# caumente/multi_task_breast_cancer

Hardware: AMD Instinct MI355X
Metric: training images/sec (1-ch 256x256, U-Net++ MT) (higher is better)
Workload: dtype bf16; 1 GPU; MTUNetPlusPlus seg+cls deep-supervision step (Dice+Focal, alpha=0.5, Adam eps 1e-4), per-GPU batch 32, 1x256x256, bf16 MFMA operands (3x3 convs, ConvT) and 16-bit stored conv outputs / activations; fp32 accumulation, gradient sums, statistics, losses, parameters and optimizer, random-init weights (BASELINE.json configs[1]); global_batch=32, parallelism=dp1

## Files before the change

### include/mtbc.h

```cpp
#ifndef MTBC_H
#define MTBC_H

#include <stddef.h>
#include <stdint.h>

#ifdef __cplusplus
extern "C" {
#endif

#define MTBC_VERSION 202
#define MTBC_MAX_SEGS 6

enum {
    MTBC_OK = 0,
    MTBC_E_BADSHAPE = -1,
    MTBC_E_BADARG = -2,
    MTBC_E_WORKSPACE = -3,
    MTBC_E_LAUNCH = -4,
    MTBC_E_UNSUPPORTED = -5
};

int mtbc_version(void);
const char* mtbc_strerror(int code);
const char* mtbc_arch(void);
// ... 163 lines not shown
    int32_t accumulate_dw;
    void* workspace; size_t workspace_bytes;
    int32_t compute;
    int32_t y_layout;
    int32_t y_type;
    int32_t x_layout;
    int32_t dy_type16;
    int32_t x_type16;
} mtbc_convT_args;
int mtbc_convT_fwd_c8_supported(const mtbc_convT_args* a);

size_t mtbc_convT_wgrad_workspace(const mtbc_convT_args* a);
int mtbc_convT_fwd(const mtbc_convT_args* a, void* stream);
int mtbc_convT_dgrad(const mtbc_convT_args* a, void* stream);
int mtbc_convT_wgrad(const mtbc_convT_args* a, void* stream);

typedef struct {
    int32_t N, H, W, Cin, Cout;
    const float* x;  int64_t x_batch_stride;
    const float* w;
    const float* bias;
    float* y;
    const float* dy;
    float* dx;       int64_t dx_batch_stride;
    int32_t accumulate_dx;
    float* dw;       float* dbias;
    int32_t accumulate_dw;
    void* workspace; size_t workspace_bytes;
    int32_t x_layout;
    int32_t x_type;
// ... 179 lines not shown
```

### multi_task_breast_cancer_amd/_lib.py

```python
from __future__ import annotations

import ctypes as C
import os
from typing import Optional

_HERE = os.path.dirname(os.path.abspath(__file__))
LIB_PATH = os.environ.get("MTBC_LIB") or os.path.join(_HERE, "libmtbc_hip.so")

MAX_SEGS = 6
c_float_p = C.POINTER(C.c_float)


class MtbcError(RuntimeError):
    pass


LAYOUT_PLANAR, LAYOUT_C8 = 0, 1


class Seg(C.Structure):
    _fields_ = [("ptr", C.c_void_p), ("batch_stride", C.c_int64), ("channels", C.c_int32), ("accumulate", C.c_int32)]


class Conv3x3Args(C.Structure):
# ... 194 lines not shown
    _fields_ = [("w", C.c_void_p), ("packed", C.c_void_p), ("Cin", C.c_int32), ("Cout", C.c_int32),
                ("kind", C.c_int32), ("compute", C.c_int32)]


class WViewDesc(C.Structure):
    _fields_ = [("w", C.c_void_p), ("dst", C.c_void_p), ("Cout", C.c_int32), ("Cin", C.c_int32), ("ci_off", C.c_int32),
                ("ci_cnt", C.c_int32), ("mode", C.c_int32), ("k_off", C.c_int32), ("K", C.c_int32)]


EXPORTS = [
    "mtbc_version", "mtbc_strerror", "mtbc_arch",
    "mtbc_conv3x3_packed_elems", "mtbc_conv3x3_packed_dgrad_elems", "mtbc_conv3x3_pack_fwd",
    "mtbc_conv3x3_pack_dgrad", "mtbc_conv3x3_packed_lp_elems", "mtbc_conv3x3_pack_lp", "mtbc_conv3x3_pack_many", "mtbc_c8_pack", "mtbc_c8_unpack", "mtbc_c8_pack16", "mtbc_conv3x3_weight_view", "mtbc_conv3x3_weight_view_many", "mtbc_augment_flip_rotate", "mtbc_convT_head_combine", "mtbc_convT_head_expand", "mtbc_conv3x3_wgrad_workspace", "mtbc_conv3x3_wgrad_sync_bytes", "mtbc_conv3x3_stats_slots", "mtbc_conv3x3_kernel_name", "mtbc_conv3x3_fwd", "mtbc_conv3x3_dgrad",
    "mtbc_conv3x3_wgrad", "mtbc_instnorm_fwd_workspace", "mtbc_instnorm_coop_state_bytes", "mtbc_instnorm_coop_error_offset", "mtbc_instnorm_c8_supported", "mtbc_instnorm_bwd_team", "mtbc_instnorm_dparam_many", "mtbc_instnorm_lrelu_fwd", "mtbc_instnorm_lrelu_bwd", "mtbc_maxpool2_fwd",
    "mtbc_maxpool2_bwd", "mtbc_convT_wgrad_workspace", "mtbc_convT_fwd_c8_supported", "mtbc_convT_fwd", "mtbc_convT_dgrad", "mtbc_convT_wgrad",
    "mtbc_conv1x1_wgrad_workspace", "mtbc_conv1x1_fwd", "mtbc_conv1x1_dgrad", "mtbc_conv1x1_wgrad",
    "mtbc_gap_fwd", "mtbc_gap_bwd", "mtbc_linear_fwd", "mtbc_linear_bwd", "mtbc_dice_fwd", "mtbc_dice_bwd",
    "mtbc_focal_fwd_bwd", "mtbc_loss_mix", "mtbc_adam_step", "mtbc_adam_dynamic", "mtbc_loss_scale_begin", "mtbc_loss_scale_check", "mtbc_loss_scale_adam",
    "mtbc_loss_scale_update_host", "mtbc_loss_scale_begin_host", "mtbc_dice_counts", "mtbc_program_run",
    "mtbc_program_run_ms", "mtbc_event_create", "mtbc_event_destroy",
    "mtbc_seg_metrics_workspace_size", "mtbc_seg_metrics",
]

ABI_VERSION = 202
_lib: Optional[C.CDLL] = None


def load() -> C.CDLL:
    global _lib
    if _lib is not None:
# ... 32 lines not shown
    lib.mtbc_c8_pack.restype = C.c_int
    lib.mtbc_c8_pack.argtypes = [C.c_void_p, C.c_int64, C.c_void_p, C.c_int32, C.c_int32, C.c_int32, C.c_int32, C.c_void_p]
    lib.mtbc_conv3x3_weight_view.restype = C.c_int
    lib.mtbc_conv3x3_weight_view.argtypes = [C.c_void_p, C.c_void_p] + [C.c_int32] * 7 + [C.c_void_p]
    lib.mtbc_conv3x3_weight_view_many.restype = C.c_int
    lib.mtbc_conv3x3_weight_view_many.argtypes = [C.POINTER(WViewDesc), C.c_int32, C.c_void_p]
    lib.mtbc_c8_pack16.restype = C.c_int
    lib.mtbc_c8_pack16.argtypes = [C.c_void_p, C.c_int64, C.c_void_p, C.c_int32, C.c_int32, C.c_int32, C.c_void_p]
    lib.mtbc_c8_unpack.restype = C.c_int
    lib.mtbc_c8_unpack.argtypes = [C.c_void_p, C.c_void_p, C.c_int32, C.c_int32, C.c_int32, C.c_int32, C.c_void_p]
    lib.mtbc_conv3x3_pack_lp.restype = C.c_int
    lib.mtbc_conv3x3_pack_lp.argtypes = [C.c_void_p, C.c_void_p, C.c_int32, C.c_int32, C.c_int32, C.c_int32, C.c_void_p]
    for name in ("mtbc_conv3x3_pack_fwd", "mtbc_conv3x3_pack_dgrad"):
        getattr(lib, name).restype = C.c_int
        getattr(lib, name).argtypes = [C.c_void_p, C.c_void_p, C.c_int32, C.c_int32, C.c_void_p]
    for name, typ in (("mtbc_conv3x3_wgrad_workspace", Conv3x3Args), ("mtbc_conv3x3_wgrad_sync_bytes", Conv3x3Args), ("mtbc_convT_wgrad_workspace", ConvTArgs),
                      ("mtbc_conv1x1_wgrad_workspace", Conv1x1Args)):
        getattr(lib, name).restype = C.c_size_t
        getattr(lib, name).argtypes = [C.POINTER(typ)]
    for name, typ in (("mtbc_conv3x3_fwd", Conv3x3Args), ("mtbc_conv3x3_dgrad", Conv3x3Args),
                      ("mtbc_conv3x3_wgrad", Conv3x3Args), ("mtbc_instnorm_lrelu_fwd", InstNormArgs),
                      ("mtbc_instnorm_lrelu_bwd", InstNormArgs), ("mtbc_maxpool2_fwd", MaxPoolArgs),
                      ("mtbc_maxpool2_bwd", MaxPoolArgs), ("mtbc_convT_fwd", ConvTArgs),
                      ("mtbc_convT_dgrad", ConvTArgs), ("mtbc_convT_wgrad", ConvTArgs),
                      ("mtbc_conv1x1_fwd", Conv1x1Args), ("mtbc_conv1x1_dgrad", Conv1x1Args),
                      ("mtbc_conv1x1_wgrad", Conv1x1Args), ("mtbc_gap_fwd", GapArgs), ("mtbc_gap_bwd", GapArgs),
                      ("mtbc_linear_fwd", LinearArgs), ("mtbc_linear_bwd", LinearArgs),
                      ("mtbc_dice_fwd", DiceArgs), ("mtbc_dice_bwd", DiceArgs), ("mtbc_focal_fwd_bwd", FocalArgs),
                      ("mtbc_adam_step", AdamArgs)):
        getattr(lib, name).restype = C.c_int
        getattr(lib, name).argtypes = [C.POINTER(typ), C.c_void_p]
    lib.mtbc_instnorm_coop_state_bytes.restype = C.c_size_t
    lib.mtbc_instnorm_coop_state_bytes.argtypes = []
    lib.mtbc_instnorm_coop_error_offset.restype = C.c_size_t
    lib.mtbc_instnorm_coop_error_offset.argtypes = []
    lib.mtbc_instnorm_bwd_team.restype = C.c_int32
    lib.mtbc_instnorm_bwd_team.argtypes = [C.POINTER(InstNormArgs)]
    lib.mtbc_instnorm_dparam_many.restype = C.c_int
    lib.mtbc_instnorm_dparam_many.argtypes = [C.POINTER(DparamDesc), C.c_int32, C.c_void_p]
    lib.mtbc_instnorm_c8_supported.restype = C.c_int
    lib.mtbc_instnorm_c8_supported.argtypes = [C.POINTER(InstNormArgs), C.c_int32]
    lib.mtbc_convT_fwd_c8_supported.restype = C.c_int
    lib.mtbc_convT_fwd_c8_supported.argtypes = [C.POINTER(ConvTArgs)]
    lib.mtbc_loss_mix.restype = C.c_int
    lib.mtbc_loss_mix.argtypes = [C.c_void_p, C.c_void_p, C.c_float, C.c_void_p, C.c_void_p]
    lib.mtbc_dice_counts.restype = C.c_int
    lib.mtbc_dice_counts.argtypes = [C.c_void_p, C.c_void_p, C.c_int64, C.c_void_p, C.c_void_p]
    lib.mtbc_adam_dynamic.restype = C.c_int
    lib.mtbc_adam_dynamic.argtypes = [C.POINTER(AdamArgs), C.POINTER(C.c_float * 3)]
    for name in ("mtbc_loss_scale_begin", "mtbc_loss_scale_check"):
        getattr(lib, name).restype = C.c_int
        getattr(lib, name).argtypes = [C.POINTER(LossScaleArgs), C.c_void_p]
    lib.mtbc_loss_scale_adam.restype = C.c_int
    lib.mtbc_loss_scale_adam.argtypes = [C.POINTER(LossScaleArgs), C.POINTER(AdamArgs), C.c_void_p]
    for name in ("mtbc_loss_scale_update_host", "mtbc_loss_scale_begin_host"):
        getattr(lib, name).restype = C.c_int
        getattr(lib, name).argtypes = [C.POINTER(LossScaleArgs)]
    lib.mtbc_program_run.restype = C.c_int
# ... 27 lines not shown
```

### multi_task_breast_cancer_amd/csrc/common.h

```cpp
#pragma once
#include <hip/hip_runtime.h>
#include <stdint.h>
#include "../../include/mtbc.h"

#define MTBC_WAVE 64

typedef float f32x4 __attribute__((ext_vector_type(4)));

#define MTBC_CHECK_LAUNCH()                                   \
    do {                                                      \
        hipError_t e__ = hipGetLastError();                   \
        if (e__ != hipSuccess) return MTBC_E_LAUNCH;          \
    } while (0)

#ifdef MTBC_PROBES
#include <stdlib.h>
static inline int mtbc_probe_int(const char* name, int dflt) { const char* v = getenv(name); return v ? atoi(v) : dflt; }
static inline bool mtbc_probe_set(const char* name) { return getenv(name) != nullptr; }
#define MTBC_DBG_BIT(p, bit) ((p).dbg & (bit))
#else
#define mtbc_probe_int(name, dflt) (dflt)
#define mtbc_probe_set(name) (false)
#define MTBC_DBG_BIT(p, bit) (0)
#endif
// ... 100 lines not shown
int mtbc_i_maxpool_c8_bwd(const mtbc_maxpool_args* a, hipStream_t st);
int mtbc_i_conv1x1_c8_fwd(const mtbc_conv1x1_args* a, hipStream_t st);
size_t mtbc_i_conv1x1_c8_wgrad_workspace(const mtbc_conv1x1_args* a);
int mtbc_i_conv1x1_c8_wgrad(const mtbc_conv1x1_args* a, hipStream_t st);
int mtbc_i_splitk_reduce(const float* partial, float* out, int nsplit, size_t elems, int accumulate, hipStream_t st);
int mtbc_i_splitk_reduce2(const float* partial, float* out, float* out2, int nsplit, size_t elems1, size_t elems2, int accumulate, hipStream_t st);
bool mtbc_i_convT2_fwd_ok(const mtbc_convT_args* a);
int mtbc_i_convT2_fwd(const mtbc_convT_args* a, hipStream_t st);
bool mtbc_i_convT2_fwd_c8_ok(const mtbc_convT_args* a);
int mtbc_i_convT2_fwd_c8(const mtbc_convT_args* a, hipStream_t st);
bool mtbc_i_convT2_fwd_lp_c8_ok(const mtbc_convT_args* a);
int mtbc_i_convT2_fwd_lp_c8(const mtbc_convT_args* a, hipStream_t st);
bool mtbc_i_convT2_dgrad_ok(const mtbc_convT_args* a);
bool mtbc_i_convT2_wgrad_ok(const mtbc_convT_args* a);
void mtbc_i_convT2_wgrad_plan(const mtbc_convT_args* a, int* steps_per_split, int* nsplit);
int mtbc_i_convT2_dgrad(const mtbc_convT_args* a, int compute, hipStream_t st);
int mtbc_i_convT2_wgrad(const mtbc_convT_args* a, int compute, float* partial, float* dbias_part, int steps_per_split, int nsplit, hipStream_t st);
int mtbc_i_channel_sums(const float* x, float* planes_ws, float* out, int N, int C, int HW, int accumulate, hipStream_t st);
```

### multi_task_breast_cancer_amd/csrc/convt2.hip

```cpp
#include "common.h"
#include <utility>

namespace {

typedef __bf16 bf16x8 __attribute__((ext_vector_type(8)));
typedef _Float16 f16x8 __attribute__((ext_vector_type(8)));

template <int LP> struct Frag;
template <> struct Frag<0> {
    float v[8];
    __device__ __forceinline__ void set(const float* f) {
#pragma unroll
        for (int i = 0; i < 8; ++i) v[i] = f[i];
    }
    static __device__ __forceinline__ f32x4 mma(const Frag& a, const Frag& b, f32x4 c) {
#pragma unroll
        for (int i = 0; i < 8; ++i) c = __builtin_amdgcn_mfma_f32_16x16x4f32(a.v[i], b.v[i], c, 0, 0, 0);
        return c;
    }
};
template <> struct Frag<1> {
    bf16x8 v;
    __device__ __forceinline__ void set(const float* f) {
#pragma unroll
// ... 770 lines not shown
            for (int m = 0; m < MT; ++m)
#pragma unroll
                for (int r = 0; r < 4; ++r) old[m][r] = *reinterpret_cast<const float2*>(dxn + (size_t)min(mb * 48 + m * 16 + kg * 4 + r, p.Cin - 1) * HW);
        }
#pragma unroll
        for (int m = 0; m < MT; ++m)
#pragma unroll
            for (int r = 0; r < 4; ++r) {
                const int ci = mb * 48 + m * 16 + kg * 4 + r;
                if (ci >= p.Cin) continue;
                float2 v = make_float2(acc[m][0][r], acc[m][1][r]);
                if (p.acc_dx) { v.x += old[m][r].x; v.y += old[m][r].y; }
                *reinterpret_cast<float2*>(dxn + (size_t)ci * HW) = v;
            }
    }
}

bool al16(const void* q) { return (reinterpret_cast<uintptr_t>(q) & 15) == 0; }

void fill(const mtbc_convT_args* a, Ct2P* p) {
    p->N = a->N; p->H = a->H; p->W = a->W; p->Cin = a->Cin; p->Cout = a->Cout;
    p->x = a->x; p->xbs = a->x_batch_stride; p->w = a->w; p->dy = a->dy; p->dybs = a->dy_batch_stride;
    p->dx = a->dx; p->dxbs = a->dx_batch_stride; p->acc_dx = a->accumulate_dx; p->partial = nullptr; p->dbias_part = nullptr;
    p->mblocks = cdiv(a->Cin, 48); p->ctiles = cdiv(a->Cout, 8); p->steps_per_split = 1; p->nsplit = 1; p->ntasks = 0; p->xcd_tasks = 0;
}

}

bool mtbc_i_convT2_dgrad_ok(const mtbc_convT_args* a) {
    const int HW = a->H * a->W;
// ... 169 lines not shown
            else hipLaunchKernelGGL((convT2_wgrad16_kernel<2, 2, 4>), dim3(b2), dim3(256), 0, st, p);
        } else {
            const unsigned b1 = xblocks ? xblocks : blocks;
            if (compute == 1) hipLaunchKernelGGL((convT2_wgrad16_kernel<1, 1, 4>), dim3(b1), dim3(256), 0, st, p);
            else hipLaunchKernelGGL((convT2_wgrad16_kernel<2, 1, 4>), dim3(b1), dim3(256), 0, st, p);
        }
    } else if (a->dy_type16) {
        if (compute == 1) hipLaunchKernelGGL((convT2_wgrad_kernel<1, true>), dim3(blocks), dim3(256), 0, st, p);
        else hipLaunchKernelGGL((convT2_wgrad_kernel<2, true>), dim3(blocks), dim3(256), 0, st, p);
    } else if (compute == 1) hipLaunchKernelGGL(convT2_wgrad_kernel<1>, dim3(blocks), dim3(256), 0, st, p);
    else if (compute == 2) hipLaunchKernelGGL(convT2_wgrad_kernel<2>, dim3(blocks), dim3(256), 0, st, p);
    else hipLaunchKernelGGL(convT2_wgrad_kernel<0>, dim3(blocks), dim3(256), 0, st, p);
    MTBC_CHECK_LAUNCH();
    return MTBC_OK;
}
```

### multi_task_breast_cancer_amd/csrc/pool_up.hip

```cpp
#include "common.h"
#include <cstdlib>

namespace {

constexpr int GRS = 81;

template <bool A_KCONTIG, bool B_KCONTIG, class AL, class BL, class CS>
__device__ __forceinline__ void gemm_block_64x64(int m0, int c0, int kbeg, int kend, AL al, BL bl, CS cs) {
    constexpr int BK = 32;
    __shared__ float As[BK * GRS];
    __shared__ float Bs[BK * GRS];
    const int tid = threadIdx.x, lane = tid & 63, wv = tid >> 6;
    const int j = lane & 15, kk = lane >> 4;
    const int mrow = 32 * (wv >> 1), ccol = 32 * (wv & 1);
    f32x4 acc[2][2];
#pragma unroll
    for (int a = 0; a < 2; ++a)
#pragma unroll
        for (int b = 0; b < 2; ++b) acc[a][b] = (f32x4){0.f, 0.f, 0.f, 0.f};

    float ra[8], rb[8];
    auto fetch = [&](int k0) {
#pragma unroll
        for (int i = 0; i < 8; ++i) {
// ... 356 lines not shown
        if (a->k == 2) hipLaunchKernelGGL(convT_wgrad_kernel<2>, grid, dim3(256), 0, st, p);
        else if (a->k == 4) hipLaunchKernelGGL(convT_wgrad_kernel<4>, grid, dim3(256), 0, st, p);
        else hipLaunchKernelGGL(convT_wgrad_kernel<8>, grid, dim3(256), 0, st, p);
        MTBC_CHECK_LAUNCH();
    }
    const size_t wel = (size_t)a->Cin * p.M;
    rc = mtbc_i_splitk_reduce(p.partial, a->dw, nsplit, wel, a->accumulate_dw, st); if (rc) return rc;
    if (a->dbias && !bias_done) {
        if (p.dybs != (long long)a->Cout * a->H * a->W * a->k * a->k) return MTBC_E_UNSUPPORTED;
        rc = mtbc_i_channel_sums(p.dy, p.partial + (size_t)nsplit * wel, a->dbias, a->N, a->Cout, a->H * a->W * a->k * a->k,
                                 a->accumulate_dw, st);
        if (rc) return rc;
    }
    return MTBC_OK;
}

static int fill_mp(const mtbc_maxpool_args* a, MpP* p) {
    if (!a || a->N <= 0 || a->C <= 0 || a->H < 2 || a->W < 2 || (a->H & 1) || (a->W & 1)) return MTBC_E_BADSHAPE;
    p->N = a->N; p->C = a->C; p->H = a->H; p->W = a->W; p->x = a->x; p->xbs = a->x_batch_stride; p->y = a->y;
    p->ybs = a->y_batch_stride; p->dy = a->dy; p->dybs = a->dy_batch_stride; p->dx = a->dx; p->dxbs = a->dx_batch_stride;
    p->acc = a->accumulate_dx;
    return MTBC_OK;
}
int mtbc_maxpool2_fwd(const mtbc_maxpool_args* a, void* stream) {
    MpP p; int rc = fill_mp(a, &p); if (rc) return rc;
    if (!p.x || !p.y) return MTBC_E_BADARG;
    if (a->layout == MTBC_LAYOUT_C8) return mtbc_i_maxpool_c8_fwd(a, (hipStream_t)stream);
    if (a->layout != MTBC_LAYOUT_PLANAR) return MTBC_E_BADARG;
    hipStream_t st = (hipStream_t)stream;
    if ((a->W & 3) == 0 && al16(p.x) && (p.xbs & 3) == 0 && (reinterpret_cast<uintptr_t>(p.y) & 7) == 0 && (p.ybs & 1) == 0) {
// ... 144 lines not shown
```

### multi_task_breast_cancer_amd/csrc/program.hip

```cpp
#include "common.h"

extern "C" {

int mtbc_version(void) { return MTBC_VERSION; }
const char* mtbc_arch(void) { return "gfx950"; }

const char* mtbc_strerror(int code) {
    switch (code) {
        case MTBC_OK: return "ok";
        case MTBC_E_BADSHAPE: return "bad shape";
        case MTBC_E_BADARG: return "bad argument (null or misaligned pointer)";
        case MTBC_E_WORKSPACE: return "workspace missing or too small";
        case MTBC_E_LAUNCH: return "kernel launch failed";
        case MTBC_E_UNSUPPORTED: return "unsupported configuration";
        default: return "unknown error";
    }
}

static inline bool is_pack(int32_t k) { return k == MTBC_OP_CONV3_PACK_FWD || k == MTBC_OP_CONV3_PACK_DGRAD || k == MTBC_OP_CONV3_PACK_LP; }

int mtbc_event_create(void** event) {
    if (!event) return MTBC_E_BADARG;
    hipEvent_t e;
    if (hipEventCreateWithFlags(&e, hipEventDisableTiming) != hipSuccess) return MTBC_E_LAUNCH;
// ... 78 lines not shown
            case MTBC_OP_CONV3_WGRAD: rc = mtbc_conv3x3_wgrad(&o->u.conv3, stream); break;
            case MTBC_OP_CONV3_PACK_FWD: rc = mtbc_conv3x3_pack_fwd(o->u.pack.w, o->u.pack.packed, o->u.pack.Cin, o->u.pack.Cout, stream); break;
            case MTBC_OP_CONV3_PACK_DGRAD: rc = mtbc_conv3x3_pack_dgrad(o->u.pack.w, o->u.pack.packed, o->u.pack.Cin, o->u.pack.Cout, stream); break;
            case MTBC_OP_HEAD_COMBINE: rc = mtbc_convT_head_combine(&o->u.head, stream); break;
            case MTBC_OP_HEAD_EXPAND: rc = mtbc_convT_head_expand(&o->u.head, stream); break;
            case MTBC_OP_CONV3_WVIEW: rc = mtbc_conv3x3_weight_view(o->u.wview.w, o->u.wview.dst, o->u.wview.Cout, o->u.wview.Cin, o->u.wview.ci_off, o->u.wview.ci_cnt, o->u.wview.mode, o->u.wview.k_off, o->u.wview.K, stream); break;
            case MTBC_OP_C8_PACK16: rc = mtbc_c8_pack16(o->u.c8pack.src, o->u.c8pack.src_batch_stride, o->u.c8pack.dst, o->u.c8pack.N, o->u.c8pack.C, o->u.c8pack.HW, stream); break;
            case MTBC_OP_C8_PACK: rc = mtbc_c8_pack(o->u.c8pack.src, o->u.c8pack.src_batch_stride, o->u.c8pack.dst, o->u.c8pack.N, o->u.c8pack.C, o->u.c8pack.HW, o->u.c8pack.compute, stream); break;
            case MTBC_OP_CONV3_PACK_LP: rc = mtbc_conv3x3_pack_lp(o->u.pack.w, o->u.pack.packed, o->u.pack.Cin, o->u.pack.Cout, o->u.pack.dgrad, o->u.pack.compute, stream); break;
            case MTBC_OP_IN_FWD: rc = mtbc_instnorm_lrelu_fwd(&o->u.inorm, stream); break;
            case MTBC_OP_IN_BWD: rc = mtbc_instnorm_lrelu_bwd(&o->u.inorm, stream); break;
            case MTBC_OP_POOL_FWD: rc = mtbc_maxpool2_fwd(&o->u.pool, stream); break;
            case MTBC_OP_POOL_BWD: rc = mtbc_maxpool2_bwd(&o->u.pool, stream); break;
            case MTBC_OP_CONVT_FWD: rc = mtbc_convT_fwd(&o->u.convT, stream); break;
            case MTBC_OP_CONVT_DGRAD: rc = mtbc_convT_dgrad(&o->u.convT, stream); break;
            case MTBC_OP_CONVT_WGRAD: rc = mtbc_convT_wgrad(&o->u.convT, stream); break;
            case MTBC_OP_CONV1_FWD: rc = mtbc_conv1x1_fwd(&o->u.conv1, stream); break;
            case MTBC_OP_CONV1_DGRAD: rc = mtbc_conv1x1_dgrad(&o->u.conv1, stream); break;
            case MTBC_OP_CONV1_WGRAD: rc = mtbc_conv1x1_wgrad(&o->u.conv1, stream); break;
            case MTBC_OP_GAP_FWD: rc = mtbc_gap_fwd(&o->u.gap, stream); break;
            case MTBC_OP_GAP_BWD: rc = mtbc_gap_bwd(&o->u.gap, stream); break;
            case MTBC_OP_LINEAR_FWD: rc = mtbc_linear_fwd(&o->u.linear, stream); break;
            case MTBC_OP_LINEAR_BWD: rc = mtbc_linear_bwd(&o->u.linear, stream); break;
            case MTBC_OP_DICE_FWD: rc = mtbc_dice_fwd(&o->u.dice, stream); break;
            case MTBC_OP_DICE_BWD: rc = mtbc_dice_bwd(&o->u.dice, stream); break;
            case MTBC_OP_FOCAL: rc = mtbc_focal_fwd_bwd(&o->u.focal, stream); break;
            case MTBC_OP_LOSS_MIX: rc = mtbc_loss_mix(o->u.mix.seg, o->u.mix.cls, o->u.mix.alpha, o->u.mix.out4, stream); break;
            case MTBC_OP_ADAM: rc = mtbc_adam_step(&o->u.adam, stream); break;
            case MTBC_OP_MEMSET:
                rc = hipMemsetAsync(o->u.memset0.ptr, 0, o->u.memset0.bytes, (hipStream_t)stream) == hipSuccess ? MTBC_OK : MTBC_E_LAUNCH;
                break;
// ... 13 lines not shown
```

### multi_task_breast_cancer_amd/engine.py

```python
from __future__ import annotations

import ctypes as C
from dataclasses import dataclass, field
from typing import Callable, Dict, List, Optional, Sequence, Tuple

import torch

from . import _lib as L


from . import switches as _sw

_sw.refuse_removed()
_NO_COOP = _sw.flag("MTBC_NO_COOP")
_NO_GATHER = _sw.flag("MTBC_NO_GATHER")
_NO_Z16 = _sw.flag("MTBC_NO_Z16")
_Z_BF16 = _sw.flag("MTBC_Z_BF16")
_DA16 = _sw.flag("MTBC_DA16")
_COOP_MIN_FWD, _COOP_MIN_BWD = 16384, 65536
_IN_KERNEL_SPLITK = False
_DPARAM_BATCH = 12


def _ptr(t: Optional[torch.Tensor]) -> Optional[int]:
    return None if t is None else t.data_ptr()


@dataclass
class Act:
    name: str
    data: torch.Tensor
    needs_grad: bool = True
# ... 711 lines not shown
            dy = y.grad16 if g16 else self.grad_of(y)
            x16 = (g16 and x.in_op is not None and bool(x.in_op.u.inorm.y8) and x.in_op.u.inorm.stats_slots > 0
                   and (x.H * x.W) % 8 == 0 and x.bstride % 8 == 0)
            op = base(reads_x=not x16)
            if x16:
                x.p16_users.append(op)
            op.kind = L.OP_CONVT_WGRAD
            a = op.u.convT
            a.compute = lp
            a.dy, a.dy_batch_stride, a.dy_type16 = dy.data_ptr(), y.bstride, (lp if g16 else 0)
            a.accumulate_dw = self._mark_param(wname)
            a.dw = self.gv(wname).data_ptr()
            if bname:
                self._mark_param(bname)
                a.dbias = self.gv(bname).data_ptr()
            self._need_ws(op, "convT", self.lib.mtbc_convT_wgrad_workspace(C.byref(a)))
            self.bwd_ops.append(op)
            if x.needs_grad:
                op = base(reads_x=False)
                op.kind = L.OP_CONVT_DGRAD
                a = op.u.convT
                a.compute = lp
                a.dy, a.dy_batch_stride, a.dy_type16 = dy.data_ptr(), y.bstride, (lp if g16 else 0)
                gx, acc = self.grad_slot(x)
                a.dx, a.dx_batch_stride, a.accumulate_dx = gx.data_ptr(), x.bstride, acc
                self.bwd_ops.append(op)

        self.bwd_emitters.append(emit_bwd)
        return y

# ... 296 lines not shown
```

### multi_task_breast_cancer_amd/ops.py

```python
from __future__ import annotations

import ctypes as C
from typing import List, Optional, Sequence, Tuple

import torch

from . import _lib as L


def _s() -> C.c_void_p:
    return C.c_void_p(torch.cuda.current_stream().cuda_stream)


def _chk(*ts):
    for t in ts:
        if t is None:
            continue
        if t.device.type != "cuda":
            L.require_gpu()
            raise L.MtbcError("device tensors required")
        if t.dtype != torch.float32 or not t.is_contiguous():
            raise ValueError("fp32 contiguous tensors required")


# ... 585 lines not shown
def convT_wgrad(x, w, dy, k, want_bias=True, compute=0, dy16=False, x16=False):
    _chk(None if x16 else x, w, None if dy16 else dy)
    dw = torch.empty_like(w)
    db = torch.empty(w.shape[1], dtype=torch.float32, device=x.device) if want_bias else None
    a = _ct_args(x, w, k)
    a.compute = compute
    a.dy_type16 = compute if dy16 else 0
    a.x_type16 = compute if x16 else 0
    a.dy, a.dy_batch_stride, a.dw, a.dbias = dy.data_ptr(), dy[0].numel(), dw.data_ptr(), _p(db)
    ws = _ws(L.load().mtbc_convT_wgrad_workspace(C.byref(a)), x.device)
    a.workspace, a.workspace_bytes = ws.data_ptr(), ws.numel() * 4
    L.check(L.load().mtbc_convT_wgrad(C.byref(a), _s()), "convT_wgrad")
    return dw, db


def _c1_args(x, w):
    a = L.Conv1x1Args()
    N, Cin, H, W = x.shape
    a.N, a.H, a.W, a.Cin, a.Cout = N, H, W, Cin, w.shape[0]
    a.x, a.x_batch_stride, a.w = x.data_ptr(), Cin * H * W, w.data_ptr()
    return a


def conv1x1_fwd(x, w, bias):
    _chk(x, w, bias)
    N, _, H, W = x.shape
    y = torch.empty(N, w.shape[0], H, W, dtype=torch.float32, device=x.device)
    a = _c1_args(x, w)
    a.bias, a.y = _p(bias), y.data_ptr()
    L.check(L.load().mtbc_conv1x1_fwd(C.byref(a), _s()), "conv1x1_fwd")
# ... 180 lines not shown
```

### multi_task_breast_cancer_amd/switches.py

```python
from __future__ import annotations

import os
from typing import Dict, List

PLAN_SWITCHES: Dict[str, tuple] = {
    "MTBC_NO_COOP": ("0", "InstanceNorm by one-plane workgroups (fp32 conv outputs) + pack instead of the channel-group / cooperative kernels: "
                          "the fallback when their teams cannot be co-resident (the cooperative error message names it)",
                     "tests/test_model_gpu.py::test_16bit_mfma_modes_match_their_emulation[...-no_coop-40]"),
    "MTBC_NO_GATHER": ("0", "every 3x3 conv back-propagates into all its inputs (fan-in by read-modify-write) instead of one gathered launch per dense-skip tensor",
                       "tests/test_model_gpu.py::test_16bit_mfma_modes_match_their_emulation[...-no_gather]"),
    "MTBC_NO_Z16": ("0", "16-bit modes keep the conv outputs z as fp32 planes (InstanceNorm reads 4 bytes per element in both directions): the storage arm of the quality sweeps",
                    "tests/test_model_gpu.py::test_16bit_mfma_modes_match_their_emulation[...-no_z16]"),
    "MTBC_Z_BF16": ("0", "bf16 mode stores the conv outputs as bf16 instead of fp16 (same bytes, 8 instead of 11 significant bits)",
                    "tests/test_model_gpu.py::test_16bit_mfma_modes_match_their_emulation[...-z_bf16]"),
    "MTBC_DA16": ("0", "the gradient a conv-cell activation gets from its 3x3 consumers is written by ONE gathered launch as a 16-bit channel-blocked tensor (fp32 sum in the MFMA "
                       "accumulators, one RNE) instead of fp32 planar fan-in: -0.36 ms per step.  Default in round 3 on the easy task's evidence (-0.010 +- 0.025 pt); OFF again since "
                       "round 4: on the task that can fail it ends at the same Dice (-0.012 +- 0.042 pt against fp32, 10 paired seeds) but reaches the plateau LATER -- mid-run "
                       "-5.6 +- 2.9 pt against fp32 where the fp32-gradient plan is at -0.5 +- 1.4 and tracks the fp32 runs seed by seed (profiles/r04_quality_hard.md)",
                  "tests/test_model_gpu.py::test_16bit_mfma_modes_match_their_emulation[...-da16]"),
    "MTBC_NOFUSE_HEADS": ("0", "MTnnUNet deep-supervision heads as ConvT + 1x1 (the reference's two layers) instead of one combined ConvT",
                          "tests/test_model_gpu.py::test_mtnnunet_two_layer_heads_match_the_fused_heads_and_the_oracle"),
    "MTBC_GRAPH": ("0", "trainer.FusedTrainStep (single process) captures each compiled step -- weight images, forward, losses, backward, Adam -- into ONE hipGraph at its third call "
                        "and replays it from then on: the host issues a step in 0.1 ms instead of 8.4 (profiles/r04_graph_replay.txt); the GPU time is the same, the results are the same bits "
                        "(Adam's per-step scalars travel through device memory, mtbc_adam_args.dynamic)",
                   "tests/test_model_gpu.py::test_graph_replayed_steps_are_the_eager_steps"),
    "MTBC_DYN_SCALE": ("0", "trainer.FusedTrainStep(loss_scale=None) trains with the device-side dynamic loss scale (loss_scale.DynamicLossScale(): start 2^16, found-inf check "
                            "over the flat gradients, skip + halve on overflow, double after 2000 clean steps) instead of the static scale baked into the loss ops: three more "
                            "launches per step; without an overflow the same bits as the static 2^16 of fp16 mode",
                       "tests/test_loss_scale_gpu.py::test_dynamic_steps_without_overflow_are_the_static_steps"),
    "MTBC_COOP_RESERVE_CUS": ("64", "CUs kept out of the cooperative InstanceNorm grids under data parallel",
                              "tests/test_coop_safety_gpu.py::test_cooperative_step_beside_a_cu_hogging_kernel"),
}
REMOVED = ("MTBC_NO_C8", "MTBC_NO_CT_LP", "MTBC_COOP_MIN_FWD", "MTBC_COOP_MIN_BWD", "MTBC_NO_P16", "MTBC_FANIN", "MTBC_NO_C8_SMALL_OPS", "MTBC_NO_X16",
           "MTBC_NO_G16", "MTBC_NO_EPI_STATS", "MTBC_EPI_BSTATS", "MTBC_NO_R1", "MTBC_NO_POOLFOLD", "MTBC_SPLIT_FANIN", "MTBC_NO_STEM16",
           "MTBC_NO_DEFER_DPARAM", "MTBC_DPARAM_BATCH", "MTBC_NO_POOLFWD_FOLD", "MTBC_BWD_OVERLAP", "MTBC_BWD_OVERLAP_MAX_HW",
           "MTBC_NO_DA16")
RESULT_ALTERING = ("MTBC_DBG", "MTBC_NOACC", "MTBC_LOWP", "MTBC_LP_MT", "MTBC_RING", "MTBC_NODMA", "MTBC_C8_BLOCKS_PER_CU",
                   "MTBC_WGRAD_LP1", "MTBC_CT_WG_TASKS", "MTBC_IN_BWD_STREAM", "MTBC_CONVT_GENERIC", "MTBC_C8_NW", "MTBC_C8_RING",
                   "MTBC_CT_DEPTH", "MTBC_CT_WG_CT", "MTBC_CT_WG_XCD", "MTBC_CT_DGRAD_DIRECT", "MTBC_WGRAD_C8W", "MTBC_C8W_BPC", "MTBC_C8W_DEPTH", "MTBC_C8W_HACK",
                   "MTBC_WGRAD_PACK24", "MTBC_WGRAD_C8I", "MTBC_WG_NS8", "MTBC_WG_TS", "MTBC_C8_TS", "MTBC_RING_TS", "MTBC_INB_TS")


def get(name: str) -> str:
    return os.environ.get(name, PLAN_SWITCHES[name][0])
# ... 28 lines not shown
```

Measured before the change: 3043 images/sec.

## Fuse ConvT k=2 weight-gradient and input-gradient into one backward kernel

Adds a combined backward kernel for the 2x2 transposed convolution with Cout=48. One launch computes dw partials and dx, reading dy once and staging the weights in LDS, with dgrad MFMA work interleaved with the wgrad pipeline per wave. The engine uses it by default when the shape is supported, in place of the separate wgrad and dgrad launches. It adds a specialised kernel, only one output-channel width qualifies, and dw/dbias may differ in fp32 summation order.

After: 3065 images/sec (median of 6 runs). No clear change (+0.7%).

```diff
diff --git a/include/mtbc.h b/include/mtbc.h
--- a/include/mtbc.h
+++ b/include/mtbc.h
@@ -201,6 +201,9 @@
 int mtbc_convT_fwd(const mtbc_convT_args* a, void* stream);
 int mtbc_convT_dgrad(const mtbc_convT_args* a, void* stream);
 int mtbc_convT_wgrad(const mtbc_convT_args* a, void* stream);
+int mtbc_convT_backward_supported(const mtbc_convT_args* a);
+size_t mtbc_convT_backward_workspace(const mtbc_convT_args* a);
+int mtbc_convT_backward(const mtbc_convT_args* a, void* stream);
 
 typedef struct {
     int32_t N, H, W, Cin, Cout;
diff --git a/multi_task_breast_cancer_amd/_lib.py b/multi_task_breast_cancer_amd/_lib.py
--- a/multi_task_breast_cancer_amd/_lib.py
+++ b/multi_task_breast_cancer_amd/_lib.py
@@ -232,6 +232,7 @@
     "mtbc_conv3x3_pack_dgrad", "mtbc_conv3x3_packed_lp_elems", "mtbc_conv3x3_pack_lp", "mtbc_conv3x3_pack_many", "mtbc_c8_pack", "mtbc_c8_unpack", "mtbc_c8_pack16", "mtbc_conv3x3_weight_view", "mtbc_conv3x3_weight_view_many", "mtbc_augment_flip_rotate", "mtbc_convT_head_combine", "mtbc_convT_head_expand", "mtbc_conv3x3_wgrad_workspace", "mtbc_conv3x3_wgrad_sync_bytes", "mtbc_conv3x3_stats_slots", "mtbc_conv3x3_kernel_name", "mtbc_conv3x3_fwd", "mtbc_conv3x3_dgrad",
     "mtbc_conv3x3_wgrad", "mtbc_instnorm_fwd_workspace", "mtbc_instnorm_coop_state_bytes", "mtbc_instnorm_coop_error_offset", "mtbc_instnorm_c8_supported", "mtbc_instnorm_bwd_team", "mtbc_instnorm_dparam_many", "mtbc_instnorm_lrelu_fwd", "mtbc_instnorm_lrelu_bwd", "mtbc_maxpool2_fwd",
     "mtbc_maxpool2_bwd", "mtbc_convT_wgrad_workspace", "mtbc_convT_fwd_c8_supported", "mtbc_convT_fwd", "mtbc_convT_dgrad", "mtbc_convT_wgrad",
+    "mtbc_convT_backward_supported", "mtbc_convT_backward_workspace", "mtbc_convT_backward",
     "mtbc_conv1x1_wgrad_workspace", "mtbc_conv1x1_fwd", "mtbc_conv1x1_dgrad", "mtbc_conv1x1_wgrad",
     "mtbc_gap_fwd", "mtbc_gap_bwd", "mtbc_linear_fwd", "mtbc_linear_bwd", "mtbc_dice_fwd", "mtbc_dice_bwd",
     "mtbc_focal_fwd_bwd", "mtbc_loss_mix", "mtbc_adam_step", "mtbc_adam_dynamic", "mtbc_loss_scale_begin", "mtbc_loss_scale_check", "mtbc_loss_scale_adam",
@@ -294,7 +295,7 @@
     for name in ("mtbc_conv3x3_pack_fwd", "mtbc_conv3x3_pack_dgrad"):
         getattr(lib, name).restype = C.c_int
         getattr(lib, name).argtypes = [C.c_void_p, C.c_void_p, C.c_int32, C.c_int32, C.c_void_p]
-    for name, typ in (("mtbc_conv3x3_wgrad_workspace", Conv3x3Args), ("mtbc_conv3x3_wgrad_sync_bytes", Conv3x3Args), ("mtbc_convT_wgrad_workspace", ConvTArgs),
+    for name, typ in (("mtbc_conv3x3_wgrad_workspace", Conv3x3Args), ("mtbc_conv3x3_wgrad_sync_bytes", Conv3x3Args), ("mtbc_convT_wgrad_workspace", ConvTArgs), ("mtbc_convT_backward_workspace", ConvTArgs),
                       ("mtbc_conv1x1_wgrad_workspace", Conv1x1Args)):
         getattr(lib, name).restype = C.c_size_t
         getattr(lib, name).argtypes = [C.POINTER(typ)]
@@ -302,7 +303,7 @@
                       ("mtbc_conv3x3_wgrad", Conv3x3Args), ("mtbc_instnorm_lrelu_fwd", InstNormArgs),
                       ("mtbc_instnorm_lrelu_bwd", InstNormArgs), ("mtbc_maxpool2_fwd", MaxPoolArgs),
                       ("mtbc_maxpool2_bwd", MaxPoolArgs), ("mtbc_convT_fwd", ConvTArgs),
-                      ("mtbc_convT_dgrad", ConvTArgs), ("mtbc_convT_wgrad", ConvTArgs),
+                      ("mtbc_convT_dgrad", ConvTArgs), ("mtbc_convT_wgrad", ConvTArgs), ("mtbc_convT_backward", ConvTArgs),
                       ("mtbc_conv1x1_fwd", Conv1x1Args), ("mtbc_conv1x1_dgrad", Conv1x1Args),
                       ("mtbc_conv1x1_wgrad", Conv1x1Args), ("mtbc_gap_fwd", GapArgs), ("mtbc_gap_bwd", GapArgs),
                       ("mtbc_linear_fwd", LinearArgs), ("mtbc_linear_bwd", LinearArgs),
@@ -322,6 +323,8 @@
     lib.mtbc_instnorm_c8_supported.argtypes = [C.POINTER(InstNormArgs), C.c_int32]
     lib.mtbc_convT_fwd_c8_supported.restype = C.c_int
     lib.mtbc_convT_fwd_c8_supported.argtypes = [C.POINTER(ConvTArgs)]
+    lib.mtbc_convT_backward_supported.restype = C.c_int
+    lib.mtbc_convT_backward_supported.argtypes = [C.POINTER(ConvTArgs)]
     lib.mtbc_loss_mix.restype = C.c_int
     lib.mtbc_loss_mix.argtypes = [C.c_void_p, C.c_void_p, C.c_float, C.c_void_p, C.c_void_p]
     lib.mtbc_dice_counts.restype = C.c_int
diff --git a/multi_task_breast_cancer_amd/csrc/common.h b/multi_task_breast_cancer_amd/csrc/common.h
--- a/multi_task_breast_cancer_amd/csrc/common.h
+++ b/multi_task_breast_cancer_amd/csrc/common.h
@@ -138,6 +138,8 @@
 bool mtbc_i_convT2_dgrad_ok(const mtbc_convT_args* a);
 bool mtbc_i_convT2_wgrad_ok(const mtbc_convT_args* a);
 void mtbc_i_convT2_wgrad_plan(const mtbc_convT_args* a, int* steps_per_split, int* nsplit);
+bool mtbc_i_convT2_bwd_ok(const mtbc_convT_args* a);
+int mtbc_i_convT2_bwd(const mtbc_convT_args* a, float* partial, float* dbias_part, int prow, int steps_per_split, int nsplit, hipStream_t st);
 int mtbc_i_convT2_dgrad(const mtbc_convT_args* a, int compute, hipStream_t st);
 int mtbc_i_convT2_wgrad(const mtbc_convT_args* a, int compute, float* partial, float* dbias_part, int steps_per_split, int nsplit, hipStream_t st);
 int mtbc_i_channel_sums(const float* x, float* planes_ws, float* out, int N, int C, int HW, int accumulate, hipStream_t st);
diff --git a/multi_task_breast_cancer_amd/csrc/convt2.hip b/multi_task_breast_cancer_amd/csrc/convt2.hip
--- a/multi_task_breast_cancer_amd/csrc/convt2.hip
+++ b/multi_task_breast_cancer_amd/csrc/convt2.hip
@@ -808,6 +808,207 @@
                 *reinterpret_cast<float2*>(dxn + (size_t)ci * HW) = v;
             }
     }
+}
+
+constexpr int BW_CO = 48, BW_WPS = BW_CO / 8, BW_WROW = 4 * BW_CO + 16, BW_NT = 64 * BW_WPS;
+template <int LP, bool X16, bool ACC>
+__global__ __launch_bounds__(BW_NT) void convT2_bwd48_kernel(const Ct2P p, const int prow) {
+    static_assert(LP != 0, "16-bit operands");
+    __shared__ __attribute__((aligned(16))) unsigned short Wd[48 * BW_WROW];
+    const int tid = threadIdx.x, lane = tid & 63, wq = __builtin_amdgcn_readfirstlane(tid >> 6);
+    const int j = lane & 15, kg = lane >> 4;
+    const int split = blockIdx.x, mb = blockIdx.y;
+    const int HW = p.H * p.W, oW = 2 * p.W;
+    constexpr int M4 = 4 * BW_CO, ppr = M4 / 8, npieces = 48 * ppr;
+    for (int base = tid; base < npieces; base += BW_NT * 4) {
+        float4 v[4][2];
+#pragma unroll
+        for (int u = 0; u < 4; ++u) {
+            const int idx = min(base + BW_NT * u, npieces - 1), r = idx / ppr, q = idx - r * ppr;
+            const float* src = p.w + (size_t)min(mb * 48 + r, p.Cin - 1) * M4 + 8 * q;
+            v[u][0] = ld4(src); v[u][1] = ld4(src + 4);
+        }
+#pragma unroll
+        for (int u = 0; u < 4; ++u) {
+            const int idx = base + BW_NT * u;
+            if (idx >= npieces) continue;
+            const int r = idx / ppr, q = idx - r * ppr;
+            ct_u32x4 o = {cvt_pk16<LP == 2>(v[u][0].x, v[u][0].y), cvt_pk16<LP == 2>(v[u][0].z, v[u][0].w),
+                          cvt_pk16<LP == 2>(v[u][1].x, v[u][1].y), cvt_pk16<LP == 2>(v[u][1].z, v[u][1].w)};
+            if (mb * 48 + r >= p.Cin) o = (ct_u32x4){0u, 0u, 0u, 0u};
+            *reinterpret_cast<ct_u32x4*>(Wd + (size_t)r * BW_WROW + 8 * q) = o;
+        }
+    }
+    __syncthreads();
+    const int spi = HW / 32, total_steps = p.N * spi;
+    const int g0 = split * p.steps_per_split, g1 = min(total_steps, g0 + p.steps_per_split), last = g1 - 1;
+    if (g0 >= g1) return;
+    const unsigned short* dy16 = reinterpret_cast<const unsigned short*>(p.dy);
+
+    bool rok[MT];
+    const unsigned short* xr16[MT];
+    const float* xr32[MT];
+#pragma unroll
+    for (int m = 0; m < MT; ++m) {
+        const int ci = mb * 48 + m * 16 + j;
+        rok[m] = ci < p.Cin;
+        xr16[m] = reinterpret_cast<const unsigned short*>(p.x) + (size_t)(rok[m] ? ci : 0) * HW + 8 * kg;
+        xr32[m] = p.x + (size_t)(rok[m] ? ci : 0) * HW + 8 * kg;
+    }
+    const int co = wq * 8 + (j >> 1);
+    const unsigned short* dcol = dy16 + (size_t)co * 4 * HW + (size_t)(j & 1) * oW;
+    f32x4 wacc[MT][2];
+#pragma unroll
+    for (int m = 0; m < MT; ++m) { wacc[m][0] = (f32x4){0.f, 0.f, 0.f, 0.f}; wacc[m][1] = (f32x4){0.f, 0.f, 0.f, 0.f}; }
+    const bool want_bias = p.dbias_part != nullptr && mb == 0;
+    float bsum = 0.f;
+    ct_u32x4 rx[2][MT], rh[2][2];
+    float4 ra[2][X16 ? 1 : MT][2];
+    auto wload = [&](int g, auto SL) {
+        constexpr int slot = decltype(SL)::value;
+        const int n = g / spi, st = g % spi;
+        const int pix = st * 32 + 8 * kg;
+        const int i = pix / p.W, jx = pix % p.W;
+#pragma unroll
+        for (int m = 0; m < MT; ++m) {
+            if constexpr (X16) rx[slot][m] = *reinterpret_cast<const ct_u32x4*>(xr16[m] + (size_t)n * p.xbs + st * 32);
+            else { const float* q = xr32[m] + (size_t)n * p.xbs + st * 32; ra[slot][m][0] = ld4(q); ra[slot][m][1] = ld4(q + 4); }
+        }
+        const unsigned short* q = dcol + (size_t)n * p.dybs + (size_t)(2 * i) * oW + 2 * jx;
+        rh[slot][0] = *reinterpret_cast<const ct_u32x4*>(q); rh[slot][1] = *reinterpret_cast<const ct_u32x4*>(q + 8);
+    };
+    auto wcompute = [&](auto SL) {
+        constexpr int cur = decltype(SL)::value;
+        Frag<LP> fa[MT];
+#pragma unroll
+        for (int m = 0; m < MT; ++m) {
+            if constexpr (X16) {
+                const ct_u32x4 w = rx[cur][m];
+                frag_from_words<LP>(fa[m], rok[m] ? w[0] : 0u, rok[m] ? w[1] : 0u, rok[m] ? w[2] : 0u, rok[m] ? w[3] : 0u);
+            } else {
+                float a[8];
+                a[0] = rok[m] ? ra[cur][m][0].x : 0.f; a[1] = rok[m] ? ra[cur][m][0].y : 0.f; a[2] = rok[m] ? ra[cur][m][0].z : 0.f; a[3] = rok[m] ? ra[cur][m][0].w : 0.f;
+                a[4] = rok[m] ? ra[cur][m][1].x : 0.f; a[5] = rok[m] ? ra[cur][m][1].y : 0.f; a[6] = rok[m] ? ra[cur][m][1].z : 0.f; a[7] = rok[m] ? ra[cur][m][1].w : 0.f;
+                fa[m].set(a);
+            }
+        }
+        unsigned d[8], w0[4], w1[4];
+#pragma unroll
+        for (int k = 0; k < 4; ++k) { d[k] = rh[cur][0][k]; d[4 + k] = rh[cur][1][k]; }
+#pragma unroll
+        for (int m = 0; m < 4; ++m) {
+            w0[m] = (d[2 * m] & 0xffffu) | (d[2 * m + 1] << 16);
+            w1[m] = (d[2 * m] >> 16) | (d[2 * m + 1] & 0xffff0000u);
+        }
+        if (want_bias) {
+#pragma unroll
+            for (int k = 0; k < 8; ++k) bsum += sum2_16<LP>(d[k]);
+        }
+        Frag<LP> f0, f1;
+        frag_from_words<LP>(f0, w0[0], w0[1], w0[2], w0[3]);
+        frag_from_words<LP>(f1, w1[0], w1[1], w1[2], w1[3]);
+#pragma unroll
+        for (int m = 0; m < MT; ++m) {
+            wacc[m][0] = Frag<LP>::mma(fa[m], f0, wacc[m][0]);
+            wacc[m][1] = Frag<LP>::mma(fa[m], f1, wacc[m][1]);
+        }
+    };
+
+    const unsigned short* arow = Wd + (size_t)j * BW_WROW + 8 * kg;
+    const unsigned short* dq = dy16;
+    float* dxn = p.dx;
+    f32x4 dacc[MT][2];
+    uint2 rd[BW_WPS][4];
+    float2 old[MT][4];
+    auto dsetup = [&](int g) {
+        const int n = g / spi, st = g % spi;
+        const int pix = st * 32 + 2 * j;
+        const int i = pix / p.W, jx = pix % p.W;
+        dq = dy16 + (size_t)n * p.dybs + (size_t)(2 * i) * oW + 2 * jx + (size_t)(2 * kg) * 4 * HW;
+        dxn = p.dx + (size_t)n * p.dxbs + st * 32 + 2 * j;
+#pragma unroll
+        for (int m = 0; m < MT; ++m) { dacc[m][0] = (f32x4){0.f, 0.f, 0.f, 0.f}; dacc[m][1] = (f32x4){0.f, 0.f, 0.f, 0.f}; }
+    };
+    auto dload = [&](auto SS) {
+        constexpr int s = decltype(SS)::value;
+        const unsigned short* q = dq + (size_t)(8 * s) * 4 * HW;
+#pragma unroll
+        for (int c = 0; c < 2; ++c) {
+            rd[s][2 * c] = *reinterpret_cast<const uint2*>(q + (size_t)c * 4 * HW);
+            rd[s][2 * c + 1] = *reinterpret_cast<const uint2*>(q + (size_t)c * 4 * HW + oW);
+        }
+    };
+    auto dcompute = [&](auto SS) {
+        constexpr int s = decltype(SS)::value;
+        Frag<LP> fe, fo;
+        frag_from_words<LP>(fe, rd[s][0].x, rd[s][1].x, rd[s][2].x, rd[s][3].x);
+        frag_from_words<LP>(fo, rd[s][0].y, rd[s][1].y, rd[s][2].y, rd[s][3].y);
+#pragma unroll
+        for (int m = 0; m < MT; ++m) {
+            Frag<LP> fa;
+            fa.v = __builtin_bit_cast(decltype(fa.v), *reinterpret_cast<const ct_u32x4*>(arow + (size_t)(m * 16) * BW_WROW + 32 * s));
+            dacc[m][0] = Frag<LP>::mma(fa, fe, dacc[m][0]);
+            dacc[m][1] = Frag<LP>::mma(fa, fo, dacc[m][1]);
+        }
+    };
+    auto dold = [&]() {
+#pragma unroll
+        for (int m = 0; m < MT; ++m)
+#pragma unroll
+            for (int r = 0; r < 4; ++r) old[m][r] = *reinterpret_cast<const float2*>(dxn + (size_t)min(mb * 48 + m * 16 + kg * 4 + r, p.Cin - 1) * HW);
+    };
+    auto dstore = [&]() {
+#pragma unroll
+        for (int m = 0; m < MT; ++m)
+#pragma unroll
+            for (int r = 0; r < 4; ++r) {
+                const int ci = mb * 48 + m * 16 + kg * 4 + r;
+                if (ci >= p.Cin) continue;
+                float2 v = make_float2(dacc[m][0][r], dacc[m][1][r]);
+                if constexpr (ACC) { v.x += old[m][r].x; v.y += old[m][r].y; }
+                *reinterpret_cast<float2*>(dxn + (size_t)ci * HW) = v;
+            }
+    };
+
+    auto group = [&](int gb, auto FULLT) {
+        constexpr bool full = decltype(FULLT)::value;
+        const int gd = gb + wq;
+        dsetup(min(gd, last));
+        sfor<BW_WPS>([&](auto U) {
+            constexpr int u = decltype(U)::value;
+            if constexpr (u < BW_WPS - 2) dload(U);
+            if constexpr (u == BW_WPS - 2) { dload(SC<BW_WPS - 2>{}); dload(SC<BW_WPS - 1>{}); }
+            if constexpr (u == BW_WPS - 1 && ACC) dold();
+            wload(min(gb + u + 1, last), SC<(u + 1) & 1>{});
+            __builtin_amdgcn_sched_barrier(0);
+            if (full || gb + u < g1) wcompute(SC<(u & 1)>{});
+            if constexpr (u >= 1) dcompute(SC<(u >= 1 ? u - 1 : 0)>{});
+            __builtin_amdgcn_sched_barrier(0);
+        });
+        dcompute(SC<BW_WPS - 1>{});
+        if (full || gd < g1) dstore();
+    };
+    wload(g0, S0{});
+    int gb = g0;
+    for (; gb + BW_WPS <= g1; gb += BW_WPS) group(gb, std::true_type{});
+    if (gb < g1) group(gb, std::false_type{});
+
+    if (want_bias) {
+        float b = bsum;
+        b += __shfl_xor(b, 16);
+        b += __shfl_xor(b, 32);
+        b += __shfl_xor(b, 1);
+        if (kg == 0 && (j & 1) == 0) p.dbias_part[(size_t)split * prow + co] = b;
+    }
+    float* part = p.partial + (size_t)split * prow;
+#pragma unroll
+    for (int m = 0; m < MT; ++m)
+#pragma unroll
+        for (int r = 0; r < 4; ++r) {
+            const int ci = mb * 48 + m * 16 + kg * 4 + r;
+            if (ci >= p.Cin) continue;
+            *reinterpret_cast<float2*>(part + ((size_t)ci * BW_CO + co) * 4 + 2 * (j & 1)) = make_float2(wacc[m][0][r], wacc[m][1][r]);
+        }
 }
 
 bool al16(const void* q) { return (reinterpret_cast<uintptr_t>(q) & 15) == 0; }
@@ -1007,3 +1208,24 @@
     MTBC_CHECK_LAUNCH();
     return MTBC_OK;
 }
+
+bool mtbc_i_convT2_bwd_ok(const mtbc_convT_args* a) {
+    return a->k == 2 && (a->compute == 1 || a->compute == 2) && a->dy_type16 == a->compute && (a->x_type16 == 0 || a->x_type16 == a->compute) &&
+           a->Cout == BW_CO && mtbc_i_convT2_dgrad_ok(a) && mtbc_i_convT2_wgrad_ok(a);
+}
+int mtbc_i_convT2_bwd(const mtbc_convT_args* a, float* partial, float* dbias_part, int prow, int steps_per_split, int nsplit, hipStream_t st) {
+    Ct2P p; fill(a, &p);
+    p.partial = partial; p.dbias_part = dbias_part; p.steps_per_split = steps_per_split; p.nsplit = nsplit;
+    const dim3 grid((unsigned)nsplit, (unsigned)p.mblocks);
+#define MTBC_CT2BW(LP_, X16_, ACC_) hipLaunchKernelGGL((convT2_bwd48_kernel<LP_, X16_, ACC_>), grid, dim3(BW_NT), 0, st, p, prow)
+#define MTBC_CT2BW_LP(LP_)                                                                                                   \
+    do {                                                                                                                     \
+        if (a->x_type16) { if (a->accumulate_dx) MTBC_CT2BW(LP_, true, true); else MTBC_CT2BW(LP_, true, false); }           \
+        else { if (a->accumulate_dx) MTBC_CT2BW(LP_, false, true); else MTBC_CT2BW(LP_, false, false); }                     \
+    } while (0)
+    if (a->compute == 1) MTBC_CT2BW_LP(1); else MTBC_CT2BW_LP(2);
+#undef MTBC_CT2BW_LP
+#undef MTBC_CT2BW
+    MTBC_CHECK_LAUNCH();
+    return MTBC_OK;
+}
diff --git a/multi_task_breast_cancer_amd/csrc/pool_up.hip b/multi_task_breast_cancer_amd/csrc/pool_up.hip
--- a/multi_task_breast_cancer_amd/csrc/pool_up.hip
+++ b/multi_task_breast_cancer_amd/csrc/pool_up.hip
@@ -394,6 +394,35 @@
     }
     return MTBC_OK;
 }
+int mtbc_convT_backward_supported(const mtbc_convT_args* a) {
+    CtP p;
+    if (!a || fill_ct(a, &p)) return 0;
+    return mtbc_i_convT2_bwd_ok(a) ? 1 : 0;
+}
+size_t mtbc_convT_backward_workspace(const mtbc_convT_args* a) {
+    size_t need = mtbc_convT_wgrad_workspace(a);
+    if (mtbc_convT_backward_supported(a)) {
+        int sps, ns; mtbc_i_convT2_wgrad_plan(a, &sps, &ns);
+        const size_t fused = (size_t)ns * ((size_t)a->Cin * a->Cout * 4 + (a->dbias ? a->Cout : 0)) * sizeof(float);
+        if (fused > need) need = fused;
+    }
+    return need;
+}
+int mtbc_convT_backward(const mtbc_convT_args* a, void* stream) {
+    CtP p; int rc = fill_ct(a, &p); if (rc) return rc;
+    if (!a->dw) return MTBC_E_BADARG;
+    if (!a->dx) return mtbc_convT_wgrad(a, stream);
+    if (!mtbc_i_convT2_bwd_ok(a)) return MTBC_E_UNSUPPORTED;
+    if (!p.x || !p.dy || !p.w) return MTBC_E_BADARG;
+    if (!a->workspace || a->workspace_bytes < mtbc_convT_backward_workspace(a)) return MTBC_E_WORKSPACE;
+    hipStream_t st = (hipStream_t)stream;
+    int sps, nsplit; mtbc_i_convT2_wgrad_plan(a, &sps, &nsplit);
+    const size_t wel = (size_t)a->Cin * p.M;
+    const int prow = (int)(wel + (a->dbias ? (size_t)a->Cout : 0));
+    float* partial = reinterpret_cast<float*>(a->workspace);
+    rc = mtbc_i_convT2_bwd(a, partial, a->dbias ? partial + wel : nullptr, prow, sps, nsplit, st); if (rc) return rc;
+    return mtbc_i_splitk_reduce2(partial, a->dw, a->dbias, nsplit, wel, a->dbias ? (size_t)a->Cout : 0, a->accumulate_dw, st);
+}
 
 static int fill_mp(const mtbc_maxpool_args* a, MpP* p) {
     if (!a || a->N <= 0 || a->C <= 0 || a->H < 2 || a->W < 2 || (a->H & 1) || (a->W & 1)) return MTBC_E_BADSHAPE;
diff --git a/multi_task_breast_cancer_amd/csrc/program.hip b/multi_task_breast_cancer_amd/csrc/program.hip
--- a/multi_task_breast_cancer_amd/csrc/program.hip
+++ b/multi_task_breast_cancer_amd/csrc/program.hip
@@ -116,7 +116,9 @@
             case MTBC_OP_POOL_BWD: rc = mtbc_maxpool2_bwd(&o->u.pool, stream); break;
             case MTBC_OP_CONVT_FWD: rc = mtbc_convT_fwd(&o->u.convT, stream); break;
             case MTBC_OP_CONVT_DGRAD: rc = mtbc_convT_dgrad(&o->u.convT, stream); break;
-            case MTBC_OP_CONVT_WGRAD: rc = mtbc_convT_wgrad(&o->u.convT, stream); break;
+            case MTBC_OP_CONVT_WGRAD:
+                rc = o->u.convT.dx ? mtbc_convT_backward(&o->u.convT, stream) : mtbc_convT_wgrad(&o->u.convT, stream);
+                break;
             case MTBC_OP_CONV1_FWD: rc = mtbc_conv1x1_fwd(&o->u.conv1, stream); break;
             case MTBC_OP_CONV1_DGRAD: rc = mtbc_conv1x1_dgrad(&o->u.conv1, stream); break;
             case MTBC_OP_CONV1_WGRAD: rc = mtbc_conv1x1_wgrad(&o->u.conv1, stream); break;
diff --git a/multi_task_breast_cancer_amd/engine.py b/multi_task_breast_cancer_amd/engine.py
--- a/multi_task_breast_cancer_amd/engine.py
+++ b/multi_task_breast_cancer_amd/engine.py
@@ -16,6 +16,7 @@
 _NO_GATHER = _sw.flag("MTBC_NO_GATHER")
 _NO_Z16 = _sw.flag("MTBC_NO_Z16")
 _Z_BF16 = _sw.flag("MTBC_Z_BF16")
+_NO_CT_FUSE = _sw.flag("MTBC_NO_CT_FUSE")
 _DA16 = _sw.flag("MTBC_DA16")
 _COOP_MIN_FWD, _COOP_MIN_BWD = 16384, 65536
 _IN_KERNEL_SPLITK = False
@@ -757,6 +758,15 @@
             if bname:
                 self._mark_param(bname)
                 a.dbias = self.gv(bname).data_ptr()
+            if x.needs_grad and not _NO_CT_FUSE:
+                a.dx, a.dx_batch_stride = self.grad_of(x).data_ptr(), x.bstride
+                if self.lib.mtbc_convT_backward_supported(C.byref(a)):
+                    gx, a.accumulate_dx = self.grad_slot(x)
+                    assert gx.data_ptr() == a.dx
+                    self._need_ws(op, "convT", self.lib.mtbc_convT_backward_workspace(C.byref(a)))
+                    self.bwd_ops.append(op)
+                    return
+                a.dx, a.dx_batch_stride = None, 0
             self._need_ws(op, "convT", self.lib.mtbc_convT_wgrad_workspace(C.byref(a)))
             self.bwd_ops.append(op)
             if x.needs_grad:
diff --git a/multi_task_breast_cancer_amd/ops.py b/multi_task_breast_cancer_amd/ops.py
--- a/multi_task_breast_cancer_amd/ops.py
+++ b/multi_task_breast_cancer_amd/ops.py
@@ -623,6 +623,38 @@
     return dw, db
 
 
+def _ct_bwd_args(x, w, dy, k, compute, dy16, x16):
+    a = _ct_args(x, w, k)
+    a.compute = compute
+    a.dy_type16 = compute if dy16 else 0
+    a.x_type16 = compute if x16 else 0
+    a.dy, a.dy_batch_stride = dy.data_ptr(), dy[0].numel()
+    return a
+
+
+def convT_backward_supported(x, w, dy, k, compute=0, dy16=False, x16=False) -> bool:
+    return bool(L.load().mtbc_convT_backward_supported(C.byref(_ct_bwd_args(x, w, dy, k, compute, dy16, x16))))
+
+
+def convT_backward(x, w, dy, k, want_bias=True, compute=0, dy16=False, x16=False, dx=None, accumulate_dx=False, dw=None, dbias=None,
+                   accumulate_dw=False, want_dx=True):
+    _chk(None if x16 else x, w, None if dy16 else dy, dx, dw, dbias)
+    if dw is None:
+        dw = torch.empty_like(w)
+    if dbias is None and want_bias:
+        dbias = torch.empty(w.shape[1], dtype=torch.float32, device=w.device)
+    a = _ct_bwd_args(x, w, dy, k, compute, dy16, x16)
+    if want_dx:
+        if dx is None:
+            dx = torch.empty(x.shape, dtype=torch.float32, device=x.device)
+        a.dx, a.dx_batch_stride, a.accumulate_dx = dx.data_ptr(), dx[0].numel(), int(accumulate_dx)
+    a.dw, a.dbias, a.accumulate_dw = dw.data_ptr(), _p(dbias if want_bias else None), int(accumulate_dw)
+    ws = _ws(L.load().mtbc_convT_backward_workspace(C.byref(a)), w.device)
+    a.workspace, a.workspace_bytes = ws.data_ptr(), ws.numel() * 4
+    L.check(L.load().mtbc_convT_backward(C.byref(a), _s()), "convT_backward")
+    return (dx if want_dx else None), dw, (dbias if want_bias else None)
+
+
 def _c1_args(x, w):
     a = L.Conv1x1Args()
     N, Cin, H, W = x.shape
diff --git a/multi_task_breast_cancer_amd/switches.py b/multi_task_breast_cancer_amd/switches.py
--- a/multi_task_breast_cancer_amd/switches.py
+++ b/multi_task_breast_cancer_amd/switches.py
@@ -28,6 +28,10 @@
                             "over the flat gradients, skip + halve on overflow, double after 2000 clean steps) instead of the static scale baked into the loss ops: three more "
                             "launches per step; without an overflow the same bits as the static 2^16 of fp16 mode",
                        "tests/test_loss_scale_gpu.py::test_dynamic_steps_without_overflow_are_the_static_steps"),
+    "MTBC_NO_CT_FUSE": ("0", "the backward of a k = 2 up-convolution is planned as the weight-gradient launch followed by the input-gradient launch (dy read twice, two "
+                             "reductions) instead of ONE launch that reads dy once (mtbc_convT_backward, where mtbc_convT_backward_supported takes the shape): the same dx "
+                             "bits, dw / dbias up to the fp32 order of the split sums",
+                        "tests/test_convt_backward_gpu.py::test_step_with_fused_convT_backward_is_the_step_with_the_pair"),
     "MTBC_COOP_RESERVE_CUS": ("64", "CUs kept out of the cooperative InstanceNorm grids under data parallel",
                               "tests/test_coop_safety_gpu.py::test_cooperative_step_beside_a_cu_hogging_kernel"),
 }
```
